# zju3dv/object_nerf

Hardware: NVIDIA H100
Metric: rays/s (higher is better)
Workload: dtype bf16

## Files before the change

object_nerf_b200/csrc/field_pe.cuh:

```cuda
#pragma once
#include "tc_common.cuh"

namespace tc {

__device__ __forceinline__ uint32_t a_chunk_addr(uint32_t base, int row, int chunk) {
  return base + (uint32_t)(chunk >> 3) * ATOM_BYTES + (uint32_t)row * 128u + (uint32_t)(((chunk & 7) ^ (row & 7)) << 4);
}
__device__ __forceinline__ void st_chunk(uint32_t addr, uint32_t a, uint32_t b, uint32_t c, uint32_t d) {
  asm volatile("st.shared.v4.b32 [%0], {%1, %2, %3, %4};" ::"r"(addr), "r"(a), "r"(b), "r"(c), "r"(d) : "memory");
}

__device__ __forceinline__ void pe8_to_chunks(uint32_t xbase, int row, int chunk0, int stride, const float* f) {
  float s[8], c[8];
  st_chunk(a_chunk_addr(xbase, row, chunk0), pack_bf16(f[0], f[1]), pack_bf16(f[2], f[3]), pack_bf16(f[4], f[5]),
           pack_bf16(f[6], f[7]));
#pragma unroll
  for (int j = 0; j < 8; ++j) __sincosf(f[j], &s[j], &c[j]);
#pragma unroll
  for (int k = 0; k < 6; ++k) {
    st_chunk(a_chunk_addr(xbase, row, chunk0 + stride * (1 + 2 * k)), pack_bf16(s[0], s[1]), pack_bf16(s[2], s[3]),
             pack_bf16(s[4], s[5]), pack_bf16(s[6], s[7]));
    st_chunk(a_chunk_addr(xbase, row, chunk0 + stride * (2 + 2 * k)), pack_bf16(c[0], c[1]), pack_bf16(c[2], c[3]),
             pack_bf16(c[4], c[5]), pack_bf16(c[6], c[7]));
    if (k < 5) {
#pragma unroll
      for (int j = 0; j < 8; ++j) {
        const float s2 = 2.0f * s[j] * c[j];
        c[j] = fmaf(-2.0f * s[j], s[j], 1.0f);
        s[j] = s2;
      }
    }
  }
}

__device__ __forceinline__ void pe_xyz_to_chunks(uint32_t xbase, int row, int chunk0, float x, float y, float z) {
  uint32_t pk[32];
  float pend = 0.0f;
  int pos = 0;
  auto emit = [&](float val) {
    if ((pos & 1) == 0) pend = val;
    else pk[pos >> 1] = pack_bf16(pend, val);
    ++pos;
  };
  emit(x); emit(y); emit(z);
  float s[3], c[3];
  sincosf(x, &s[0], &c[0]);
  sincosf(y, &s[1], &c[1]);
  sincosf(z, &s[2], &c[2]);
#pragma unroll
  for (int k = 0; k < 10; ++k) {
    emit(s[0]); emit(s[1]); emit(s[2]);
    emit(c[0]); emit(c[1]); emit(c[2]);
    if (k < 9) {
#pragma unroll
      for (int j = 0; j < 3; ++j) {
        const float s2 = 2.0f * s[j] * c[j];
        c[j] = fmaf(-2.0f * s[j], s[j], 1.0f);
        s[j] = s2;
      }
    }
  }
  emit(0.0f);
#pragma unroll
  for (int q = 0; q < 8; ++q)
    st_chunk(a_chunk_addr(xbase, row, chunk0 + q), pk[4 * q], pk[4 * q + 1], pk[4 * q + 2], pk[4 * q + 3]);
}


}
```

object_nerf_b200/csrc/field_tc.cu:

```cuda
#include <cuda_bf16.h>

#include "encode.cuh"
#include "field_common.cuh"
#include "tc_chain.cuh"
#include "field_pe.cuh"

namespace {

using namespace tc;

constexpr float kLeaky = 0.01f;

enum Epi { EPI_HIDDEN = 0, EPI_HIDDEN_RC = 1, EPI_HIDDEN_SIGMA = 2, EPI_FINAL = 3, EPI_DIR = 4 };

struct TcParams {
  FieldParams f;
  WLayer layers[MAX_LAYERS];
  int n_layers;
  uint8_t* dump;
  TrainLayout TL;
  uint32_t* diag;
};

struct RowMeta {
  int ray, si, mute, live;
};

struct Rows {
  int row[2];
  int live[2];
  int ray[2], si[2], mute[2];
  const float* rc[2];
  int64_t tile;
};

__device__ __forceinline__ uint32_t leaky_bf16x2(uint32_t x) {
  __nv_bfloat162 v = *reinterpret_cast<__nv_bfloat162*>(&x);
  const __nv_bfloat162 slope = __floats2bfloat162_rn(kLeaky, kLeaky);
  v = __hmax2(v, __hmul2(v, slope));
  return *reinterpret_cast<uint32_t*>(&v);
}

template <int N>
__device__ __forceinline__ void dump_layer(const TcParams& P, const Rows& R, int slot, int mask_word0, const uint32_t* pk) {
  const int q = threadIdx.x & 3;
#pragma unroll
  for (int r = 0; r < 2; ++r) {
    const int row = R.row[r];
    uint8_t* base = P.dump + P.TL.act_off[slot] + ((size_t)R.tile * P.TL.act_atoms[slot]) * ATOM_BYTES + (size_t)row * 128 + q * 4;
#pragma unroll
    for (int j = 0; j < N / 8; ++j)
      *reinterpret_cast<uint32_t*>(base + (size_t)(j >> 3) * ATOM_BYTES + (((j & 7) ^ (row & 7)) << 4)) = pk[2 * j + r];
  }
  if (mask_word0 < 0) return;
  constexpr int CPW = N >= 128 ? 32 : 16, NW = N / CPW, BPW = CPW / 8;
  uint32_t* mrow = reinterpret_cast<uint32_t*>(P.dump + P.TL.mask_off) + ((size_t)R.tile * ONERF_MASK_WORDS + mask_word0) * 128;
#pragma unroll
  for (int w = 0; w < NW; ++w) {
#pragma unroll
    for (int r = 0; r < 2; ++r) {
      uint32_t m = 0;
#pragma unroll
      for (int jj = 0; jj < BPW; ++jj) {
        const uint32_t v = pk[2 * (w * BPW + jj) + r];
        const uint32_t bits = (((v >> 15) & 1u) ^ 1u) | ((((v >> 31) & 1u) ^ 1u) << 1);
        m |= bits << (8 * jj + 2 * q);
      }
      m |= __shfl_xor_sync(0xffffffffu, m, 1);
      m |= __shfl_xor_sync(0xffffffffu, m, 2);
      if (q == 0) mrow[w * 128 + R.row[r]] = m;
    }
  }
}

template <int N, int EPI>
__device__ __forceinline__ void epilogue(const float (&acc)[N / 2], uint32_t* pk, const float* bias, const Rows& R,
                                         int rc_base, const float* headw, float (&part)[2][4]) {
  const int q = threadIdx.x & 3;
#pragma unroll
  for (int j = 0; j < N / 8; ++j) {
    const int c = 8 * j + 2 * q;
    float2 b[2];
    if (EPI == EPI_HIDDEN_RC || EPI == EPI_DIR) {
      b[0] = __ldg(reinterpret_cast<const float2*>(R.rc[0] + rc_base + c));
      b[1] = __ldg(reinterpret_cast<const float2*>(R.rc[1] + rc_base + c));
    } else {
      b[0] = b[1] = *reinterpret_cast<const float2*>(bias + c);
    }
#pragma unroll
    for (int r = 0; r < 2; ++r) {
      float t0 = acc[4 * j + 2 * r] + b[r].x, t1 = acc[4 * j + 2 * r + 1] + b[r].y;
      uint32_t p;
      if (EPI == EPI_HIDDEN || EPI == EPI_HIDDEN_RC) {
        p = leaky_bf16x2(pack_bf16(t0, t1));
      } else if (EPI == EPI_FINAL) {
        p = pack_bf16(t0, t1);
      } else {
        t0 = fmaxf(t0, t0 * kLeaky);
        t1 = fmaxf(t1, t1 * kLeaky);
        if (EPI == EPI_HIDDEN_SIGMA) {
          const float2 w = __ldg(reinterpret_cast<const float2*>(headw + c));
          part[r][0] = fmaf(t1, w.y, fmaf(t0, w.x, part[r][0]));
        } else {
#pragma unroll
          for (int k = 0; k < 3; ++k) {
            const float2 w = __ldg(reinterpret_cast<const float2*>(headw + k * N + c));
            part[r][1 + k] = fmaf(t1, w.y, fmaf(t0, w.x, part[r][1 + k]));
          }
        }
        p = pack_bf16(t0, t1);
      }
      pk[2 * j + r] = p;
    }
  }
}

__device__ __forceinline__ void write_heads(const FieldParams& p, const Rows& R, int branch, float (&part)[2][4]) {
  const float* Pf = reinterpret_cast<const float*>(p.packed);
  const float* hb = Pf + (branch ? p.L.orgb_b : p.L.rgb_b);
  const float sb = __ldg(Pf + (branch ? p.L.osigma_b : p.L.sigma_b));
#pragma unroll
  for (int r = 0; r < 2; ++r) {
#pragma unroll
    for (int k = 0; k < 4; ++k) {
      part[r][k] += __shfl_xor_sync(0xffffffffu, part[r][k], 1);
      part[r][k] += __shfl_xor_sync(0xffffffffu, part[r][k], 2);
    }
    if ((threadIdx.x & 3) == 0 && R.live[r]) {
      float sg = part[r][0] + sb;
      const float cr = 1.0f / (1.0f + __expf(-(part[r][1] + __ldg(hb + 0))));
      const float cg = 1.0f / (1.0f + __expf(-(part[r][2] + __ldg(hb + 1))));
      const float cb = 1.0f / (1.0f + __expf(-(part[r][3] + __ldg(hb + 2))));
      if (R.mute[r] & (branch ? 2 : 1)) sg = -1e5f;
      float* outp = branch ? p.obj_out : p.scene_out;
      reinterpret_cast<float4*>(outp)[(int64_t)R.ray[r] * p.out_stride + R.si[r]] = make_float4(cr, cg, cb, sg);
    }
  }
}

template <bool VOXEL, bool DUMP>
__global__ void __launch_bounds__(NUM_THREADS, 1) field_tc_kernel(const __grid_constant__ TcParams P) {
  extern __shared__ __align__(1024) uint8_t smem_raw[];
  const FieldParams& p = P.f;
  const int warp = threadIdx.x >> 5, lane = threadIdx.x & 31;
  constexpr int X_ATOMS = VOXEL ? 6 : 1;
  constexpr int XS = VOXEL ? 9 : 2, XO = VOXEL ? 12 : 2;

  const uint32_t sbase = (smem_u32(smem_raw) + 1023u) & ~1023u;
  const uint32_t sX = sbase;
  const uint32_t sB = sX + X_ATOMS * ATOM_BYTES;
  const uint32_t sBias = sB + NSTAGE * STAGE_BYTES;
  const uint32_t sMeta = sBias + G_COUNT * 256 * 4;
  const uint32_t sBar = sMeta + TM * sizeof(RowMeta);
  uint8_t* gen_base = smem_raw + (sbase - smem_u32(smem_raw));
  float* bias_tab = reinterpret_cast<float*>(gen_base + (sBias - sbase));
  RowMeta* meta = reinterpret_cast<RowMeta*>(gen_base + (sMeta - sbase));
  const float* Pf = reinterpret_cast<const float*>(p.packed);
  Ring ring{sB, sBar, sBar + 8 * NSTAGE, 0u, 0u, P.diag};

  if (threadIdx.x == 0) ring_init_bars(ring.full, ring.empty);
  for (int i = threadIdx.x; i < G_COUNT * 256; i += NUM_THREADS) {
    const int g = i >> 8, c = i & 255;
    bias_tab[i] = (c < p.L.g[g].N) ? __ldg(Pf + p.L.g[g].bias_off + c) : 0.0f;
  }
  __syncthreads();

  const int64_t total = (int64_t)p.n_rays * p.S;
  const int64_t n_tiles = (total + TM - 1) / TM;

  if (warp >= PRODUCER_WARP) {
    setmaxnreg_dec<PRODUCER_REGS>();
    if (warp == PRODUCER_WARP)
      tc_producer_loop(P.layers, P.n_layers, reinterpret_cast<const uint8_t*>(p.packed), ring, n_tiles);
    return;
  }
  setmaxnreg_inc<CONSUMER_REGS>();

  const int wg = warp >> 2, tid = threadIdx.x & 127;
  const uint32_t sXw = sX + (uint32_t)wg * 64u * 128u;
  Rows R;
  R.row[0] = wg * 64 + (warp & 3) * 16 + (lane >> 2);
  R.row[1] = R.row[0] + 8;
  for (int64_t tile = blockIdx.x; tile < n_tiles; tile += gridDim.x) {
    R.tile = tile;
#pragma unroll 1
    for (int job = tid; job < 256; job += 128) {
      const int row = wg * 64 + (job & 63), cq = job >> 6;
      const int64_t e = tile * TM + row;
      const bool live = e < total;
      const int ray = live ? (int)(e / p.S) : 0;
      const int si = live ? (int)(e - (int64_t)ray * p.S) : 0;
      const float* rr = p.rays + (int64_t)ray * 8;
      const float zz = live ? __ldg(p.z + (int64_t)ray * p.z_stride + si) : 0.0f;
      float x = fmaf(__ldg(rr + 3), zz, __ldg(rr + 0));
      float y = fmaf(__ldg(rr + 4), zz, __ldg(rr + 1));
      float z = fmaf(__ldg(rr + 5), zz, __ldg(rr + 2));
      if (p.xyz && live) {
        const float* qq = p.xyz + ((int64_t)ray * p.S + si) * 3;
        x = __ldg(qq); y = __ldg(qq + 1); z = __ldg(qq + 2);
      }
      if (!live) { x = 0.f; y = 0.f; z = 0.f; }
      if (cq == 0) {
        int mute = 0;
        if (live && p.mute_zero_rays && __ldg(p.z + (int64_t)ray * p.z_stride + (p.S - 1)) == 0.0f) mute = 3;
        if (live && mute == 0 && p.n_boxes > 0 && point_in_boxes(p.boxes, p.n_boxes, x, y, z)) mute = 1;
        meta[row] = RowMeta{ray, si, mute, live ? 1 : 0};
      }
      if (VOXEL) {
        const GridView g = load_grid_view(p.grid);
        float f[8];
        if (cq == 0) {
          voxel_trilinear<0, 8, false>(g, x, y, z, f);
          pe8_to_chunks(sX, row, 0, 2, f);
        } else if (cq == 1) {
          voxel_trilinear<8, 8, false>(g, x, y, z, f);
          pe8_to_chunks(sX, row, 1, 2, f);
        } else if (cq == 2) {
          voxel_trilinear<16, 8, false>(g, x, y, z, f);
          pe8_to_chunks(sX, row, 34, 1, f);
        } else {
          pe_xyz_to_chunks(sX, row, 26, x, y, z);
          st_chunk(a_chunk_addr(sX, row, 47), 0u, 0u, 0u, 0u);
        }
      } else {
        if (cq == 0) pe_xyz_to_chunks(sX, row, 0, x, y, z);
      }
    }
    fence_async_smem();
    wg_sync(wg);
    if (DUMP) {
#pragma unroll 1
      for (int a = 0; a < X_ATOMS; ++a) {
        const uint4* src = reinterpret_cast<const uint4*>(gen_base + (size_t)a * ATOM_BYTES + (size_t)wg * 8192);
        uint4* dst = reinterpret_cast<uint4*>(P.dump + P.TL.act_off[0] + ((size_t)tile * X_ATOMS + a) * ATOM_BYTES + (size_t)wg * 8192);
        for (int i = tid; i < 512; i += 128) dst[i] = src[i];
      }
    }
#pragma unroll
    for (int r = 0; r < 2; ++r) {
      const RowMeta m = meta[R.row[r]];
      R.live[r] = m.live; R.ray[r] = m.ray; R.si[r] = m.si; R.mute[r] = m.mute;
      R.rc[r] = p.ray_const + (int64_t)m.ray * ONERF_RAY_CONST_FLOATS;
    }

    if (p.want_scene) {
      float acc[128];
      uint32_t h[64];
      float part[2][4] = {};
      const float* sw = Pf + p.L.sigma_w;
      mma_layer<256, XS, 0>(acc, h, sXw, ring);
      epilogue<256, EPI_HIDDEN>(acc, h, bias_tab + G_S0 * 256, R, 0, nullptr, part);
      if (DUMP) dump_layer<256>(P, R, 1, onerf_mask_word0(1), h);
#pragma unroll 1
      for (int l = 1; l < 4; ++l) {
        mma_layer<256, 0, 8>(acc, h, sXw, ring);
        epilogue<256, EPI_HIDDEN>(acc, h, bias_tab + (G_S0 + l) * 256, R, 0, nullptr, part);
        if (DUMP) dump_layer<256>(P, R, 1 + l, onerf_mask_word0(1 + l), h);
      }
      mma_layer<256, XS, 8>(acc, h, sXw, ring);
      epilogue<256, EPI_HIDDEN>(acc, h, bias_tab + G_S4 * 256, R, 0, nullptr, part);
      if (DUMP) dump_layer<256>(P, R, 5, onerf_mask_word0(5), h);
#pragma unroll 1
      for (int l = 5; l < 7; ++l) {
        mma_layer<256, 0, 8>(acc, h, sXw, ring);
        epilogue<256, EPI_HIDDEN>(acc, h, bias_tab + (G_S0 + l) * 256, R, 0, nullptr, part);
        if (DUMP) dump_layer<256>(P, R, 1 + l, onerf_mask_word0(1 + l), h);
      }
      mma_layer<256, 0, 8>(acc, h, sXw, ring);
      epilogue<256, EPI_HIDDEN_SIGMA>(acc, h, bias_tab + G_S7 * 256, R, 0, sw, part);
      if (DUMP) dump_layer<256>(P, R, 8, onerf_mask_word0(8), h);
      mma_layer<256, 0, 8>(acc, h, sXw, ring);
      epilogue<256, EPI_FINAL>(acc, h, bias_tab + G_SFIN * 256, R, 0, nullptr, part);
      if (DUMP) dump_layer<256>(P, R, 9, -1, h);
      float accd[64];
      uint32_t hd[32];
      mma_layer<128, 0, 8>(accd, h, sXw, ring);
      epilogue<128, EPI_DIR>(accd, hd, nullptr, R, RC_SDIR, Pf + p.L.rgb_w, part);
      if (DUMP) dump_layer<128>(P, R, 10, onerf_mask_word0(10), hd);
      write_heads(p, R, 0, part);
    }
    if (p.want_object) {
      float acc[64];
      uint32_t h[32];
      float part[2][4] = {};
      mma_layer<128, XO, 0>(acc, h, sXw, ring);
      epilogue<128, EPI_HIDDEN_RC>(acc, h, nullptr, R, RC_OL0, nullptr, part);
      if (DUMP) dump_layer<128>(P, R, 11, onerf_mask_word0(11), h);
      mma_layer<128, 0, 4>(acc, h, sXw, ring);
      epilogue<128, EPI_HIDDEN>(acc, h, bias_tab + G_O1 * 256, R, 0, nullptr, part);
      if (DUMP) dump_layer<128>(P, R, 12, onerf_mask_word0(12), h);
      mma_layer<128, XO, 4>(acc, h, sXw, ring);
      epilogue<128, EPI_HIDDEN_RC>(acc, h, nullptr, R, RC_OL2, nullptr, part);
      if (DUMP) dump_layer<128>(P, R, 13, onerf_mask_word0(13), h);
      mma_layer<128, 0, 4>(acc, h, sXw, ring);
      epilogue<128, EPI_HIDDEN_SIGMA>(acc, h, bias_tab + G_O3 * 256, R, 0, Pf + p.L.osigma_w, part);
      if (DUMP) dump_layer<128>(P, R, 14, onerf_mask_word0(14), h);
      mma_layer<128, 0, 4>(acc, h, sXw, ring);
      epilogue<128, EPI_FINAL>(acc, h, bias_tab + G_OFIN * 256, R, 0, nullptr, part);
      if (DUMP) dump_layer<128>(P, R, 15, -1, h);
      float accd[32];
      uint32_t hd[16];
      mma_layer<64, 0, 4>(accd, h, sXw, ring);
      epilogue<64, EPI_DIR>(accd, hd, nullptr, R, RC_ODIR, Pf + p.L.orgb_w, part);
      if (DUMP) dump_layer<64>(P, R, 16, onerf_mask_word0(16), hd);
      write_heads(p, R, 1, part);
    }
    wg_sync(wg);
  }
}

}

int onerf_launch_field_bf16(onerf_ctx* ctx, const FieldParams& fp, cudaStream_t stream) {
  const PackLayout& L = fp.L;
  TcParams P;
  memset(&P, 0, sizeof(P));
  P.f = fp;
  int n = 0;
  auto add = [&](int g) { P.layers[n++] = WLayer{L.g[g].img_off, L.g[g].N, L.g[g].K / 32}; };
  if (fp.want_scene)
    for (int g = G_S0; g <= G_SDIR; ++g) add(g);
  if (fp.want_object)
    for (int g = G_O0; g <= G_ODIR; ++g) add(g);
  P.n_layers = n;
  P.diag = ctx->tc_diag;
  const int64_t total = (int64_t)fp.n_rays * fp.S;
  const int64_t tiles = (total + TM - 1) / TM;
  if (fp.train_ws) {
    P.dump = reinterpret_cast<uint8_t*>(fp.train_ws);
    P.TL = onerf_make_train_layout(L.use_voxel, total);
  }
  const int blocks = (int)(tiles < ctx->num_sms ? tiles : ctx->num_sms);
  const int x_atoms = L.use_voxel ? 6 : 1;
  const size_t smem = 1024 + (size_t)x_atoms * ATOM_BYTES + NSTAGE * STAGE_BYTES + G_COUNT * 256 * 4 + TM * sizeof(RowMeta) +
                      16 * NSTAGE;
  auto launch = [&](auto kernel) -> int {
    ONERF_CUDA(cudaFuncSetAttribute(kernel, cudaFuncAttributeMaxDynamicSharedMemorySize, (int)smem));
    kernel<<<blocks, NUM_THREADS, smem, stream>>>(P);
    ONERF_LAUNCH_CHECK(ctx);
    return ONERF_OK;
  };
  if (L.use_voxel) return fp.train_ws ? launch(field_tc_kernel<true, true>) : launch(field_tc_kernel<true, false>);
  return fp.train_ws ? launch(field_tc_kernel<false, true>) : launch(field_tc_kernel<false, false>);
}
```

object_nerf_b200/csrc/tc_chain.cuh:

```cuda
#pragma once
#include "tc_common.cuh"

namespace tc {

constexpr int NSTAGE = 6;
constexpr int STAGE_BYTES = 16384;
constexpr int NUM_WG = 2;
constexpr int NUM_CONSUMER = NUM_WG * 128;
constexpr int PRODUCER_WARP = NUM_CONSUMER / 32;
constexpr int NUM_THREADS = NUM_CONSUMER + 128;
constexpr int PRODUCER_REGS = 40, CONSUMER_REGS = 232;
constexpr int MAX_LAYERS = 16;

struct WLayer {
  int64_t img_off;
  int N;
  int nslab;
};

struct Ring {
  uint32_t sB, full, empty;
  uint32_t stage, phase;
  uint32_t* diag;
};

__device__ __forceinline__ void ring_init_bars(uint32_t full, uint32_t empty) {
  for (int s = 0; s < NSTAGE; ++s) {
    mbar_init(full + 8 * s, 1);
    mbar_init(empty + 8 * s, NUM_CONSUMER / 32);
  }
  fence_barrier_init();
}

__device__ __forceinline__ void tc_producer_loop(const WLayer* layers, int n_layers, const uint8_t* blob, Ring r,
                                                 int64_t n_tiles) {
  for (int64_t tile = blockIdx.x; tile < n_tiles; tile += gridDim.x) {
    for (int l = 0; l < n_layers; ++l) {
      const WLayer& Ly = layers[l];
      const int spp = 256 / Ly.N;
      const uint32_t slab_bytes = (uint32_t)Ly.N * 64u;
      for (int s0 = 0; s0 < Ly.nslab; s0 += spp) {
        const int cnt = (Ly.nslab - s0 < spp) ? Ly.nslab - s0 : spp;
        mbar_wait(r.empty + 8 * r.stage, r.phase ^ 1, r.diag);
        if (elect_one()) {
          mbar_expect_tx(r.full + 8 * r.stage, (uint32_t)cnt * slab_bytes);
          tma_bulk_g2s(r.sB + r.stage * STAGE_BYTES, blob + Ly.img_off + (size_t)s0 * slab_bytes, (uint32_t)cnt * slab_bytes,
                       r.full + 8 * r.stage);
        }
        __syncwarp();
        if (++r.stage == NSTAGE) { r.stage = 0; r.phase ^= 1; }
      }
    }
  }
}

__device__ __forceinline__ void ring_release(const Ring& r, uint32_t stage) {
  asm volatile(
      "{\n\t.reg .pred p;\n\tsetp.eq.u32 p, %1, 0;\n\t@p mbarrier.arrive.shared::cta.b64 _, [%0];\n\t}" ::"r"(
          r.empty + 8 * stage),
      "r"(threadIdx.x & 31)
      : "memory");
}

template <int N, int NX, int NH, int W = N>
__device__ __forceinline__ void mma_layer(float (&acc)[N / 2], const uint32_t* hin, uint32_t sXw, Ring& r) {
  constexpr int SPP = 256 / N, NS = NX + NH;
#pragma unroll
  for (int i = 0; i < N / 2; ++i) acc[i] = 0.0f;
  uint32_t prev = 0;
#pragma unroll
  for (int s = 0; s < NS; ++s) {
    if (s % SPP == 0) mbar_wait(r.full + 8 * r.stage, r.phase, r.diag);
    const uint32_t b0 = r.sB + r.stage * STAGE_BYTES + (uint32_t)(s % SPP) * (uint32_t)N * 64u;
    wgmma_fence();
#pragma unroll
    for (int k16 = 0; k16 < 2; ++k16) {
#pragma unroll
      for (int nb = 0; nb < N / W; ++nb) {
        const uint64_t bd = desc_k_sw64(b0 + (uint32_t)nb * (uint32_t)W * 64u + (uint32_t)k16 * 32u);
        if (s < NX)
          wgmma_ss<W>(acc + nb * (W / 2),
                      desc_k_sw128(sXw + (uint32_t)(s >> 1) * ATOM_BYTES + (uint32_t)(s & 1) * 64u + (uint32_t)k16 * 32u), bd);
        else
          wgmma_rs<W>(acc + nb * (W / 2), hin + ((s - NX) * 2 + k16) * 4, bd);
      }
    }
    if (s % SPP == SPP - 1 || s == NS - 1) {
      wgmma_commit();
      if (s >= SPP) {
        wgmma_wait<1>();
        ring_release(r, prev);
      }
      prev = r.stage;
      if (++r.stage == NSTAGE) { r.stage = 0; r.phase ^= 1; }
    }
  }
  wgmma_wait<0>();
  ring_release(r, prev);
  fence_regs<N / 2>(acc);
}

}
```

object_nerf_b200/csrc/tc_common.cuh:

```cuda
#pragma once
#include <cuda_bf16.h>
#include <stdint.h>

namespace tc {

constexpr int TM = 128;
constexpr int ATOM_BYTES = 16384;

__device__ __forceinline__ uint32_t smem_u32(const void* p) { return (uint32_t)__cvta_generic_to_shared(p); }

__device__ __forceinline__ void mbar_init(uint32_t bar, uint32_t count) {
  asm volatile("mbarrier.init.shared::cta.b64 [%0], %1;" ::"r"(bar), "r"(count));
}
__device__ __forceinline__ void mbar_arrive(uint32_t bar) {
  asm volatile("mbarrier.arrive.shared::cta.b64 _, [%0];" ::"r"(bar) : "memory");
}
__device__ __forceinline__ void mbar_expect_tx(uint32_t bar, uint32_t bytes) {
  asm volatile("mbarrier.arrive.expect_tx.shared::cta.b64 _, [%0], %1;" ::"r"(bar), "r"(bytes) : "memory");
}
__device__ __forceinline__ void mbar_wait(uint32_t bar, uint32_t parity, uint32_t* diag) {
  asm volatile(
      "{\n\t.reg .pred p;\n\t.reg .u64 t0, t1;\n\t.reg .u32 b;\n\t"
      "mbarrier.try_wait.parity.shared::cta.b64 p, [%0], %1, %2;\n\t"
      "@p bra DONE;\n\t"
      "mov.u64 t0, %%clock64;\n"
      "WAIT:\n\t"
      "mbarrier.try_wait.parity.shared::cta.b64 p, [%0], %1, %2;\n\t"
      "@p bra DONE;\n\t"
      "mov.u64 t1, %%clock64;\n\t"
      "sub.u64 t1, t1, t0;\n\t"
      "setp.lt.u64 p, t1, %4;\n\t"
      "@p bra WAIT;\n\t"
      "mov.u32 b, %%ctaid.x;\n\t"
      "st.volatile.u32 [%3 + 4], b;\n\t"
      "st.volatile.u32 [%3 + 8], %0;\n\t"
      "st.volatile.u32 [%3 + 12], %1;\n\t"
      "membar.sys;\n\t"
      "st.volatile.u32 [%3], 1;\n\t"
      "membar.sys;\n\t"
      "trap;\n"
      "DONE:\n\t}"
      :
      : "r"(bar), "r"(parity), "r"(20000u), "l"(diag), "n"(4000000000ll)
      : "memory");
}
__device__ __forceinline__ void fence_barrier_init() { asm volatile("fence.mbarrier_init.release.cluster;" ::: "memory"); }
__device__ __forceinline__ void fence_async_smem() { asm volatile("fence.proxy.async.shared::cta;" ::: "memory"); }

__device__ __forceinline__ void tma_bulk_g2s(uint32_t dst, const void* src, uint32_t bytes, uint32_t bar) {
  asm volatile("cp.async.bulk.shared::cluster.global.mbarrier::complete_tx::bytes [%0], [%1], %2, [%3];" ::"r"(dst),
               "l"(src), "r"(bytes), "r"(bar)
               : "memory");
}

__device__ __forceinline__ bool elect_one() {
  uint32_t pred;
  asm volatile(
      "{\n\t.reg .pred p;\n\t"
      "elect.sync _|p, 0xffffffff;\n\t"
      "selp.u32 %0, 1, 0, p;\n\t}"
      : "=r"(pred));
  return pred != 0;
}

template <int N>
__device__ __forceinline__ void setmaxnreg_dec() { asm volatile("setmaxnreg.dec.sync.aligned.u32 %0;" ::"n"(N)); }
template <int N>
__device__ __forceinline__ void setmaxnreg_inc() { asm volatile("setmaxnreg.inc.sync.aligned.u32 %0;" ::"n"(N)); }

__device__ __forceinline__ void wg_sync(int wg) { asm volatile("bar.sync %0, 128;" ::"r"(1 + wg) : "memory"); }

__device__ __forceinline__ void wgmma_fence() { asm volatile("wgmma.fence.sync.aligned;" ::: "memory"); }
__device__ __forceinline__ void wgmma_commit() { asm volatile("wgmma.commit_group.sync.aligned;" ::: "memory"); }
template <int N>
__device__ __forceinline__ void wgmma_wait() { asm volatile("wgmma.wait_group.sync.aligned %0;" ::"n"(N) : "memory"); }

template <int NR>
__device__ __forceinline__ void fence_regs(float* d) {
#pragma unroll
  for (int i = 0; i < NR; ++i) asm volatile("" : "+f"(d[i])::"memory");
}

#define ONERF_WG_D32                                                                                                   \
  "{%0, %1, %2, %3, %4, %5, %6, %7, %8, %9, %10, %11, %12, %13, %14, %15, %16, %17, %18, %19, %20, %21, %22, %23, %24, " \
  "%25, %26, %27, %28, %29, %30, %31}"
#define ONERF_WG_OUT32(d)                                                                                              \
  "+f"((d)[0]), "+f"((d)[1]), "+f"((d)[2]), "+f"((d)[3]), "+f"((d)[4]), "+f"((d)[5]), "+f"((d)[6]), "+f"((d)[7]),      \
      "+f"((d)[8]), "+f"((d)[9]), "+f"((d)[10]), "+f"((d)[11]), "+f"((d)[12]), "+f"((d)[13]), "+f"((d)[14]),           \
      "+f"((d)[15]), "+f"((d)[16]), "+f"((d)[17]), "+f"((d)[18]), "+f"((d)[19]), "+f"((d)[20]), "+f"((d)[21]),         \
      "+f"((d)[22]), "+f"((d)[23]), "+f"((d)[24]), "+f"((d)[25]), "+f"((d)[26]), "+f"((d)[27]), "+f"((d)[28]),         \
      "+f"((d)[29]), "+f"((d)[30]), "+f"((d)[31])
#define ONERF_WG_OUT64(d) ONERF_WG_OUT32(d), ONERF_WG_OUT32((d) + 32)
#define ONERF_WG_OUT128(d) ONERF_WG_OUT64(d), ONERF_WG_OUT64((d) + 64)
#define ONERF_WG_D64 "{" \
  "%0, %1, %2, %3, %4, %5, %6, %7, %8, %9, %10, %11, %12, %13, %14, %15, " \
  "%16, %17, %18, %19, %20, %21, %22, %23, %24, %25, %26, %27, %28, %29, %30, %31, " \
  "%32, %33, %34, %35, %36, %37, %38, %39, %40, %41, %42, %43, %44, %45, %46, %47, " \
  "%48, %49, %50, %51, %52, %53, %54, %55, %56, %57, %58, %59, %60, %61, %62, %63" "}"
#define ONERF_WG_D128 "{" \
  "%0, %1, %2, %3, %4, %5, %6, %7, %8, %9, %10, %11, %12, %13, %14, %15, " \
  "%16, %17, %18, %19, %20, %21, %22, %23, %24, %25, %26, %27, %28, %29, %30, %31, " \
  "%32, %33, %34, %35, %36, %37, %38, %39, %40, %41, %42, %43, %44, %45, %46, %47, " \
  "%48, %49, %50, %51, %52, %53, %54, %55, %56, %57, %58, %59, %60, %61, %62, %63, " \
  "%64, %65, %66, %67, %68, %69, %70, %71, %72, %73, %74, %75, %76, %77, %78, %79, " \
  "%80, %81, %82, %83, %84, %85, %86, %87, %88, %89, %90, %91, %92, %93, %94, %95, " \
  "%96, %97, %98, %99, %100, %101, %102, %103, %104, %105, %106, %107, %108, %109, %110, %111, " \
  "%112, %113, %114, %115, %116, %117, %118, %119, %120, %121, %122, %123, %124, %125, %126, %127" "}"

__device__ __forceinline__ void wgmma_rs_n64(float* d, const uint32_t* a, uint64_t desc_b) {
  asm volatile(
      "{\n\t.reg .pred p;\n\tsetp.ne.b32 p, %37, 0;\n\t"
      "wgmma.mma_async.sync.aligned.m64n64k16.f32.bf16.bf16 " ONERF_WG_D32 ", {%32, %33, %34, %35}, %36, p, 1, 1, 0;\n\t}"
      : ONERF_WG_OUT32(d)
      : "r"(a[0]), "r"(a[1]), "r"(a[2]), "r"(a[3]), "l"(desc_b), "r"(1));
}
template <int TA, int TB>
__device__ __forceinline__ void wgmma_ss_n64(float* d, uint64_t desc_a, uint64_t desc_b) {
  asm volatile(
      "{\n\t.reg .pred p;\n\tsetp.ne.b32 p, %34, 0;\n\t"
      "wgmma.mma_async.sync.aligned.m64n64k16.f32.bf16.bf16 " ONERF_WG_D32 ", %32, %33, p, 1, 1, %35, %36;\n\t}"
      : ONERF_WG_OUT32(d)
      : "l"(desc_a), "l"(desc_b), "r"(1), "n"(TA), "n"(TB));
}

template <int N>
__device__ __forceinline__ void wgmma_rs(float* d, const uint32_t* a, uint64_t desc_b) {
  if constexpr (N == 64) {
    wgmma_rs_n64(d, a, desc_b);
  } else if constexpr (N == 128) {
    asm volatile(
        "{\n\t.reg .pred p;\n\tsetp.ne.b32 p, %69, 0;\n\t"
        "wgmma.mma_async.sync.aligned.m64n128k16.f32.bf16.bf16 " ONERF_WG_D64 ", {%64, %65, %66, %67}, %68, p, 1, 1, 0;\n\t}"
        : ONERF_WG_OUT64(d)
        : "r"(a[0]), "r"(a[1]), "r"(a[2]), "r"(a[3]), "l"(desc_b), "r"(1));
  } else {
    static_assert(N == 256, "wgmma_rs: N is 64, 128 or 256");
    asm volatile(
        "{\n\t.reg .pred p;\n\tsetp.ne.b32 p, %133, 0;\n\t"
        "wgmma.mma_async.sync.aligned.m64n256k16.f32.bf16.bf16 " ONERF_WG_D128 ", {%128, %129, %130, %131}, %132, p, 1, 1, 0;\n\t}"
        : ONERF_WG_OUT128(d)
        : "r"(a[0]), "r"(a[1]), "r"(a[2]), "r"(a[3]), "l"(desc_b), "r"(1));
  }
}
template <int N>
__device__ __forceinline__ void wgmma_ss(float* d, uint64_t desc_a, uint64_t desc_b) {
  if constexpr (N == 64) {
    wgmma_ss_n64<0, 0>(d, desc_a, desc_b);
  } else if constexpr (N == 128) {
    asm volatile(
        "{\n\t.reg .pred p;\n\tsetp.ne.b32 p, %66, 0;\n\t"
        "wgmma.mma_async.sync.aligned.m64n128k16.f32.bf16.bf16 " ONERF_WG_D64 ", %64, %65, p, 1, 1, 0, 0;\n\t}"
        : ONERF_WG_OUT64(d)
        : "l"(desc_a), "l"(desc_b), "r"(1));
  } else {
    static_assert(N == 256, "wgmma_ss: N is 64, 128 or 256");
    asm volatile(
        "{\n\t.reg .pred p;\n\tsetp.ne.b32 p, %130, 0;\n\t"
        "wgmma.mma_async.sync.aligned.m64n256k16.f32.bf16.bf16 " ONERF_WG_D128 ", %128, %129, p, 1, 1, 0, 0;\n\t}"
        : ONERF_WG_OUT128(d)
        : "l"(desc_a), "l"(desc_b), "r"(1));
  }
}

__device__ __forceinline__ uint64_t make_desc(uint32_t saddr, uint32_t lbo_bytes, uint32_t sbo_bytes, uint32_t layout) {
  return (uint64_t)((saddr >> 4) & 0x3FFFu) | ((uint64_t)((lbo_bytes >> 4) & 0x3FFFu) << 16) |
         ((uint64_t)((sbo_bytes >> 4) & 0x3FFFu) << 32) | ((uint64_t)layout << 62);
}
__device__ __forceinline__ uint64_t desc_k_sw128(uint32_t saddr) { return make_desc(saddr, 16, 1024, 1); }
__device__ __forceinline__ uint64_t desc_k_sw64(uint32_t saddr) { return make_desc(saddr, 16, 512, 2); }
__device__ __forceinline__ uint64_t desc_mn_sw128(uint32_t saddr, uint32_t lbo_bytes) { return make_desc(saddr, lbo_bytes, 1024, 1); }

__device__ __forceinline__ uint32_t pack_bf16(float lo, float hi) {
  __nv_bfloat162 t = __floats2bfloat162_rn(lo, hi);
  return *reinterpret_cast<uint32_t*>(&t);
}
__device__ __forceinline__ float bf16_lo(uint32_t w) { return __uint_as_float(w << 16); }
__device__ __forceinline__ float bf16_hi(uint32_t w) { return __uint_as_float(w & 0xffff0000u); }

__device__ __forceinline__ uint32_t atom_chunk_off(int row, int chunk) {
  return (uint32_t)(chunk >> 3) * ATOM_BYTES + (uint32_t)row * 128u + (uint32_t)(((chunk & 7) ^ (row & 7)) << 4);
}


}
```

Before: 1.463 million.

## Move input encoding to dedicated encoder warps with mbarrier handoff and prefetch

```diff
diff --git a/object_nerf_b200/csrc/field_pe.cuh b/object_nerf_b200/csrc/field_pe.cuh
--- a/object_nerf_b200/csrc/field_pe.cuh
+++ b/object_nerf_b200/csrc/field_pe.cuh
@@ -34,12 +34,13 @@
 }
 
 __device__ __forceinline__ void pe_xyz_to_chunks(uint32_t xbase, int row, int chunk0, float x, float y, float z) {
-  uint32_t pk[32];
+  uint32_t pk[4];
   float pend = 0.0f;
   int pos = 0;
   auto emit = [&](float val) {
     if ((pos & 1) == 0) pend = val;
-    else pk[pos >> 1] = pack_bf16(pend, val);
+    else pk[(pos >> 1) & 3] = pack_bf16(pend, val);
+    if ((pos & 7) == 7) st_chunk(a_chunk_addr(xbase, row, chunk0 + (pos >> 3)), pk[0], pk[1], pk[2], pk[3]);
     ++pos;
   };
   emit(x); emit(y); emit(z);
@@ -61,9 +62,6 @@
     }
   }
   emit(0.0f);
-#pragma unroll
-  for (int q = 0; q < 8; ++q)
-    st_chunk(a_chunk_addr(xbase, row, chunk0 + q), pk[4 * q], pk[4 * q + 1], pk[4 * q + 2], pk[4 * q + 3]);
 }
 
 
diff --git a/object_nerf_b200/csrc/field_tc.cu b/object_nerf_b200/csrc/field_tc.cu
--- a/object_nerf_b200/csrc/field_tc.cu
+++ b/object_nerf_b200/csrc/field_tc.cu
@@ -20,6 +20,9 @@
   uint8_t* dump;
   TrainLayout TL;
   uint32_t* diag;
+#ifdef ONERF_FIELD_TIMELINE
+  uint64_t* tl;
+#endif
 };
 
 struct RowMeta {
@@ -32,7 +35,30 @@
   int ray[2], si[2], mute[2];
   const float* rc[2];
   int64_t tile;
+#ifdef ONERF_FIELD_TIMELINE
+  uint64_t* tl;
+#endif
 };
+
+#ifdef ONERF_FIELD_TIMELINE
+constexpr int TL_CTAS = 8, TL_TILES = 16, TL_SLOTS = 80;
+uint64_t* g_timeline = nullptr;
+__device__ __forceinline__ void tl_put(uint64_t* tl, int slot, uint64_t v) {
+  asm volatile("{\n\t.reg .pred p;\n\tsetp.ne.u64 p, %0, 0;\n\t@p st.global.u64 [%1], %2;\n\t}" ::"l"(tl), "l"(tl + slot),
+               "l"(v)
+               : "memory");
+}
+__device__ __forceinline__ uint64_t* tl_record(const TcParams& P, int64_t tile, int wg, bool lead) {
+  const int64_t k = (tile - blockIdx.x) / gridDim.x;
+  if (!P.tl || !lead || blockIdx.x >= TL_CTAS || k >= TL_TILES) return nullptr;
+  return P.tl + (((int64_t)blockIdx.x * 3 + wg) * TL_TILES + k) * TL_SLOTS;
+}
+#define TL_AT(tl, slot) tl_put((tl), (slot), clock64())
+#define TL_PUT(tl, slot, v) tl_put((tl), (slot), (v))
+#else
+#define TL_AT(tl, slot)
+#define TL_PUT(tl, slot, v)
+#endif
 
 __device__ __forceinline__ uint32_t leaky_bf16x2(uint32_t x) {
   __nv_bfloat162 v = *reinterpret_cast<__nv_bfloat162*>(&x);
@@ -138,54 +164,69 @@
   }
 }
 
-template <bool VOXEL, bool DUMP>
-__global__ void __launch_bounds__(NUM_THREADS, 1) field_tc_kernel(const __grid_constant__ TcParams P) {
-  extern __shared__ __align__(1024) uint8_t smem_raw[];
+__device__ __forceinline__ void x_release(uint32_t x_free, bool on) {
+  asm volatile(
+      "{\n\t.reg .pred p;\n\tsetp.eq.u32 p, %1, 1;\n\t@p mbarrier.arrive.shared::cta.b64 _, [%0];\n\t}" ::"r"(x_free),
+      "r"((uint32_t)on & (uint32_t)((threadIdx.x & 31) == 0))
+      : "memory");
+}
+
+template <int N, int NX, int NH, int EPI, bool DUMP>
+__device__ __forceinline__ void run_layer(const TcParams& P, const Rows& R, Ring& ring, uint32_t sXw, float (&acc)[N / 2],
+                                          const uint32_t* hin, uint32_t* hout, const float* bias, int rc_base,
+                                          const float* headw, float (&part)[2][4], int slot, int mask_word0,
+                                          uint32_t x_free = 0, bool free_x = false) {
+  TL_AT(R.tl, 3 * slot);
+  mma_layer<N, NX, NH>(acc, hin, sXw, ring);
+  if constexpr (NX > 0) x_release(x_free, free_x);
+  TL_AT(R.tl, 3 * slot + 1);
+#ifdef ONERF_FIELD_TIMELINE
+  TL_PUT(R.tl, 55 + slot, ring.full_wait);
+  ring.full_wait = 0;
+#endif
+  epilogue<N, EPI>(acc, hout, bias, R, rc_base, headw, part);
+  if (DUMP) dump_layer<N>(P, R, slot, mask_word0, hout);
+  TL_AT(R.tl, 3 * slot + 2);
+}
+
+constexpr int NUM_ENCODER = 3 * 32;
+
+__device__ __forceinline__ void prefetch_l2(const void* ptr) {
+  asm volatile("prefetch.global.L2 [%0];" ::"l"(ptr));
+}
+
+__device__ __forceinline__ void prefetch_rows(const void* base, int64_t pitch, int64_t bytes0, int nbytes, int r0,
+                                              int r1, int et) {
+  const int lines = (nbytes + 127) >> 7;
+  for (int i = et; i < (r1 - r0 + 1) * lines; i += NUM_ENCODER)
+    prefetch_l2(reinterpret_cast<const char*>(base) + (r0 + i / lines) * pitch + bytes0 + (int64_t)(i % lines) * 128);
+}
+
+template <bool VOXEL>
+__device__ __forceinline__ void encoder_loop(const TcParams& P, uint32_t sX, RowMeta* meta, uint32_t x_full,
+                                             uint32_t x_free, int64_t n_tiles, int64_t total) {
   const FieldParams& p = P.f;
-  const int warp = threadIdx.x >> 5, lane = threadIdx.x & 31;
-  constexpr int X_ATOMS = VOXEL ? 6 : 1;
-  constexpr int XS = VOXEL ? 9 : 2, XO = VOXEL ? 12 : 2;
-
-  const uint32_t sbase = (smem_u32(smem_raw) + 1023u) & ~1023u;
-  const uint32_t sX = sbase;
-  const uint32_t sB = sX + X_ATOMS * ATOM_BYTES;
-  const uint32_t sBias = sB + NSTAGE * STAGE_BYTES;
-  const uint32_t sMeta = sBias + G_COUNT * 256 * 4;
-  const uint32_t sBar = sMeta + TM * sizeof(RowMeta);
-  uint8_t* gen_base = smem_raw + (sbase - smem_u32(smem_raw));
-  float* bias_tab = reinterpret_cast<float*>(gen_base + (sBias - sbase));
-  RowMeta* meta = reinterpret_cast<RowMeta*>(gen_base + (sMeta - sbase));
-  const float* Pf = reinterpret_cast<const float*>(p.packed);
-  Ring ring{sB, sBar, sBar + 8 * NSTAGE, 0u, 0u, P.diag};
-
-  if (threadIdx.x == 0) ring_init_bars(ring.full, ring.empty);
-  for (int i = threadIdx.x; i < G_COUNT * 256; i += NUM_THREADS) {
-    const int g = i >> 8, c = i & 255;
-    bias_tab[i] = (c < p.L.g[g].N) ? __ldg(Pf + p.L.g[g].bias_off + c) : 0.0f;
-  }
-  __syncthreads();
-
-  const int64_t total = (int64_t)p.n_rays * p.S;
-  const int64_t n_tiles = (total + TM - 1) / TM;
-
-  if (warp >= PRODUCER_WARP) {
-    setmaxnreg_dec<PRODUCER_REGS>();
-    if (warp == PRODUCER_WARP)
-      tc_producer_loop(P.layers, P.n_layers, reinterpret_cast<const uint8_t*>(p.packed), ring, n_tiles);
-    return;
-  }
-  setmaxnreg_inc<CONSUMER_REGS>();
-
-  const int wg = warp >> 2, tid = threadIdx.x & 127;
-  const uint32_t sXw = sX + (uint32_t)wg * 64u * 128u;
-  Rows R;
-  R.row[0] = wg * 64 + (warp & 3) * 16 + (lane >> 2);
-  R.row[1] = R.row[0] + 8;
-  for (int64_t tile = blockIdx.x; tile < n_tiles; tile += gridDim.x) {
-    R.tile = tile;
+  const int et = threadIdx.x - NUM_CONSUMER - 32;
+  constexpr int JOBS = VOXEL ? 4 * TM : TM;
+  uint32_t it = 0;
+  for (int64_t tile = blockIdx.x; tile < n_tiles; tile += gridDim.x, ++it) {
+#ifdef ONERF_FIELD_TIMELINE
+    uint64_t* tl = tl_record(P, tile, 2, et == 0);
+#endif
+    TL_AT(tl, 0);
+    {
+      const int64_t e0 = tile * TM, e1 = min(e0 + TM, total) - 1;
+      prefetch_rows(p.ray_const, ONERF_RAY_CONST_FLOATS * 4, 0, ONERF_RAY_CONST_FLOATS * 4, (int)(e0 / p.S),
+                    (int)(e1 / p.S), et);
+      const int64_t n0 = e0 + (int64_t)gridDim.x * TM, n1 = min(n0 + TM, total) - 1;
+      if (n0 < total) {
+        prefetch_rows(p.rays, 32, 0, 32, (int)(n0 / p.S), (int)(n1 / p.S), et);
+        prefetch_rows(p.z, p.z_stride * 4, 0, p.S * 4, (int)(n0 / p.S), (int)(n1 / p.S), et);
+      }
+    }
 #pragma unroll 1
-    for (int job = tid; job < 256; job += 128) {
-      const int row = wg * 64 + (job & 63), cq = job >> 6;
+    for (int job = et; job < JOBS; job += NUM_ENCODER) {
+      const int row = job & (TM - 1), cq = job / TM;
       const int64_t e = tile * TM + row;
       const bool live = e < total;
       const int ray = live ? (int)(e / p.S) : 0;
@@ -204,30 +245,91 @@
         int mute = 0;
         if (live && p.mute_zero_rays && __ldg(p.z + (int64_t)ray * p.z_stride + (p.S - 1)) == 0.0f) mute = 3;
         if (live && mute == 0 && p.n_boxes > 0 && point_in_boxes(p.boxes, p.n_boxes, x, y, z)) mute = 1;
+        mbar_wait(x_free, (it & 1) ^ 1, P.diag);
         meta[row] = RowMeta{ray, si, mute, live ? 1 : 0};
       }
-      if (VOXEL) {
+      if (VOXEL && cq < 3) {
         const GridView g = load_grid_view(p.grid);
         float f[8];
-        if (cq == 0) {
-          voxel_trilinear<0, 8, false>(g, x, y, z, f);
-          pe8_to_chunks(sX, row, 0, 2, f);
-        } else if (cq == 1) {
-          voxel_trilinear<8, 8, false>(g, x, y, z, f);
-          pe8_to_chunks(sX, row, 1, 2, f);
-        } else if (cq == 2) {
-          voxel_trilinear<16, 8, false>(g, x, y, z, f);
-          pe8_to_chunks(sX, row, 34, 1, f);
-        } else {
-          pe_xyz_to_chunks(sX, row, 26, x, y, z);
-          st_chunk(a_chunk_addr(sX, row, 47), 0u, 0u, 0u, 0u);
-        }
-      } else {
-        if (cq == 0) pe_xyz_to_chunks(sX, row, 0, x, y, z);
-      }
-    }
+        if (cq == 0) voxel_trilinear<0, 8, false>(g, x, y, z, f);
+        else if (cq == 1) voxel_trilinear<8, 8, false>(g, x, y, z, f);
+        else voxel_trilinear<16, 8, false>(g, x, y, z, f);
+        mbar_wait(x_free, (it & 1) ^ 1, P.diag);
+        pe8_to_chunks(sX, row, cq < 2 ? cq : 34, cq < 2 ? 2 : 1, f);
+      } else if (cq == (VOXEL ? 3 : 0)) {
+        mbar_wait(x_free, (it & 1) ^ 1, P.diag);
+        pe_xyz_to_chunks(sX, row, VOXEL ? 26 : 0, x, y, z);
+        if (VOXEL) st_chunk(a_chunk_addr(sX, row, 47), 0u, 0u, 0u, 0u);
+      }
+    }
+    mbar_wait(x_free, (it & 1) ^ 1, P.diag);
+    TL_AT(tl, 1);
     fence_async_smem();
-    wg_sync(wg);
+    mbar_arrive(x_full);
+    TL_AT(tl, 2);
+  }
+}
+
+template <bool VOXEL, bool DUMP>
+__global__ void __launch_bounds__(NUM_THREADS, 1) field_tc_kernel(const __grid_constant__ TcParams P) {
+  extern __shared__ __align__(1024) uint8_t smem_raw[];
+  const FieldParams& p = P.f;
+  const int warp = threadIdx.x >> 5, lane = threadIdx.x & 31;
+  constexpr int X_ATOMS = VOXEL ? 6 : 1;
+  constexpr int XS = VOXEL ? 9 : 2, XO = VOXEL ? 12 : 2;
+
+  const uint32_t sbase = (smem_u32(smem_raw) + 1023u) & ~1023u;
+  const uint32_t sX = sbase;
+  const uint32_t sB = sX + X_ATOMS * ATOM_BYTES;
+  const uint32_t sBias = sB + NSTAGE * STAGE_BYTES;
+  const uint32_t sMeta = sBias + G_COUNT * 256 * 4;
+  const uint32_t sBar = sMeta + TM * sizeof(RowMeta);
+  const uint32_t x_full = sBar + 16 * NSTAGE, x_free = x_full + 8;
+  uint8_t* gen_base = smem_raw + (sbase - smem_u32(smem_raw));
+  float* bias_tab = reinterpret_cast<float*>(gen_base + (sBias - sbase));
+  RowMeta* meta = reinterpret_cast<RowMeta*>(gen_base + (sMeta - sbase));
+  const float* Pf = reinterpret_cast<const float*>(p.packed);
+  Ring ring{sB, sBar, sBar + 8 * NSTAGE, 0u, 0u, P.diag};
+
+  if (threadIdx.x == 0) {
+    mbar_init(x_full, NUM_ENCODER);
+    mbar_init(x_free, NUM_CONSUMER / 32);
+    ring_init_bars(ring.full, ring.empty);
+  }
+  for (int i = threadIdx.x; i < G_COUNT * 256; i += NUM_THREADS) {
+    const int g = i >> 8, c = i & 255;
+    bias_tab[i] = (c < p.L.g[g].N) ? __ldg(Pf + p.L.g[g].bias_off + c) : 0.0f;
+  }
+  __syncthreads();
+
+  const int64_t total = (int64_t)p.n_rays * p.S;
+  const int64_t n_tiles = (total + TM - 1) / TM;
+
+  if (warp >= PRODUCER_WARP) {
+    setmaxnreg_dec<PRODUCER_REGS>();
+    if (warp == PRODUCER_WARP)
+      tc_producer_loop(P.layers, P.n_layers, reinterpret_cast<const uint8_t*>(p.packed), ring, n_tiles);
+    else
+      encoder_loop<VOXEL>(P, sX, meta, x_full, x_free, n_tiles, total);
+    return;
+  }
+  setmaxnreg_inc<CONSUMER_REGS>();
+
+  const int wg = warp >> 2, tid = threadIdx.x & 127;
+  const uint32_t sXw = sX + (uint32_t)wg * 64u * 128u;
+  const bool free_after_o2 = !p.want_scene;
+  Rows R;
+  R.row[0] = wg * 64 + (warp & 3) * 16 + (lane >> 2);
+  R.row[1] = R.row[0] + 8;
+  uint32_t it = 0;
+  for (int64_t tile = blockIdx.x; tile < n_tiles; tile += gridDim.x, ++it) {
+    R.tile = tile;
+#ifdef ONERF_FIELD_TIMELINE
+    R.tl = tl_record(P, tile, wg, tid == 0);
+#endif
+    TL_AT(R.tl, 0);
+    mbar_wait(x_full, it & 1, P.diag);
+    TL_AT(R.tl, 1);
     if (DUMP) {
 #pragma unroll 1
       for (int a = 0; a < X_ATOMS; ++a) {
@@ -242,70 +344,55 @@
       R.live[r] = m.live; R.ray[r] = m.ray; R.si[r] = m.si; R.mute[r] = m.mute;
       R.rc[r] = p.ray_const + (int64_t)m.ray * ONERF_RAY_CONST_FLOATS;
     }
-
+    TL_AT(R.tl, 2);
+
+    if (p.want_object) {
+      float acc[64];
+      uint32_t h[32];
+      float part[2][4] = {};
+      run_layer<128, XO, 0, EPI_HIDDEN_RC, DUMP>(P, R, ring, sXw, acc, h, h, nullptr, RC_OL0, nullptr, part, 11,
+                                                 onerf_mask_word0(11), x_free, false);
+      run_layer<128, 0, 4, EPI_HIDDEN, DUMP>(P, R, ring, sXw, acc, h, h, bias_tab + G_O1 * 256, 0, nullptr, part, 12,
+                                             onerf_mask_word0(12));
+      run_layer<128, XO, 4, EPI_HIDDEN_RC, DUMP>(P, R, ring, sXw, acc, h, h, nullptr, RC_OL2, nullptr, part, 13,
+                                                 onerf_mask_word0(13), x_free, free_after_o2);
+      run_layer<128, 0, 4, EPI_HIDDEN_SIGMA, DUMP>(P, R, ring, sXw, acc, h, h, bias_tab + G_O3 * 256, 0,
+                                                   Pf + p.L.osigma_w, part, 14, onerf_mask_word0(14));
+      run_layer<128, 0, 4, EPI_FINAL, DUMP>(P, R, ring, sXw, acc, h, h, bias_tab + G_OFIN * 256, 0, nullptr, part, 15, -1);
+      float accd[32];
+      uint32_t hd[16];
+      run_layer<64, 0, 4, EPI_DIR, DUMP>(P, R, ring, sXw, accd, h, hd, nullptr, RC_ODIR, Pf + p.L.orgb_w, part, 16,
+                                         onerf_mask_word0(16));
+      write_heads(p, R, 1, part);
+    }
     if (p.want_scene) {
       float acc[128];
       uint32_t h[64];
       float part[2][4] = {};
       const float* sw = Pf + p.L.sigma_w;
-      mma_layer<256, XS, 0>(acc, h, sXw, ring);
-      epilogue<256, EPI_HIDDEN>(acc, h, bias_tab + G_S0 * 256, R, 0, nullptr, part);
-      if (DUMP) dump_layer<256>(P, R, 1, onerf_mask_word0(1), h);
+      run_layer<256, XS, 0, EPI_HIDDEN, DUMP>(P, R, ring, sXw, acc, h, h, bias_tab + G_S0 * 256, 0, nullptr, part, 1,
+                                              onerf_mask_word0(1), x_free, false);
 #pragma unroll 1
-      for (int l = 1; l < 4; ++l) {
-        mma_layer<256, 0, 8>(acc, h, sXw, ring);
-        epilogue<256, EPI_HIDDEN>(acc, h, bias_tab + (G_S0 + l) * 256, R, 0, nullptr, part);
-        if (DUMP) dump_layer<256>(P, R, 1 + l, onerf_mask_word0(1 + l), h);
-      }
-      mma_layer<256, XS, 8>(acc, h, sXw, ring);
-      epilogue<256, EPI_HIDDEN>(acc, h, bias_tab + G_S4 * 256, R, 0, nullptr, part);
-      if (DUMP) dump_layer<256>(P, R, 5, onerf_mask_word0(5), h);
+      for (int l = 1; l < 4; ++l)
+        run_layer<256, 0, 8, EPI_HIDDEN, DUMP>(P, R, ring, sXw, acc, h, h, bias_tab + (G_S0 + l) * 256, 0, nullptr, part,
+                                               1 + l, onerf_mask_word0(1 + l));
+      run_layer<256, XS, 8, EPI_HIDDEN, DUMP>(P, R, ring, sXw, acc, h, h, bias_tab + G_S4 * 256, 0, nullptr, part, 5,
+                                              onerf_mask_word0(5), x_free, true);
 #pragma unroll 1
-      for (int l = 5; l < 7; ++l) {
-        mma_layer<256, 0, 8>(acc, h, sXw, ring);
-        epilogue<256, EPI_HIDDEN>(acc, h, bias_tab + (G_S0 + l) * 256, R, 0, nullptr, part);
-        if (DUMP) dump_layer<256>(P, R, 1 + l, onerf_mask_word0(1 + l), h);
-      }
-      mma_layer<256, 0, 8>(acc, h, sXw, ring);
-      epilogue<256, EPI_HIDDEN_SIGMA>(acc, h, bias_tab + G_S7 * 256, R, 0, sw, part);
-      if (DUMP) dump_layer<256>(P, R, 8, onerf_mask_word0(8), h);
-      mma_layer<256, 0, 8>(acc, h, sXw, ring);
-      epilogue<256, EPI_FINAL>(acc, h, bias_tab + G_SFIN * 256, R, 0, nullptr, part);
-      if (DUMP) dump_layer<256>(P, R, 9, -1, h);
+      for (int l = 5; l < 7; ++l)
+        run_layer<256, 0, 8, EPI_HIDDEN, DUMP>(P, R, ring, sXw, acc, h, h, bias_tab + (G_S0 + l) * 256, 0, nullptr, part,
+                                               1 + l, onerf_mask_word0(1 + l));
+      run_layer<256, 0, 8, EPI_HIDDEN_SIGMA, DUMP>(P, R, ring, sXw, acc, h, h, bias_tab + G_S7 * 256, 0, sw, part, 8,
+                                                   onerf_mask_word0(8));
+      run_layer<256, 0, 8, EPI_FINAL, DUMP>(P, R, ring, sXw, acc, h, h, bias_tab + G_SFIN * 256, 0, nullptr, part, 9, -1);
       float accd[64];
       uint32_t hd[32];
-      mma_layer<128, 0, 8>(accd, h, sXw, ring);
-      epilogue<128, EPI_DIR>(accd, hd, nullptr, R, RC_SDIR, Pf + p.L.rgb_w, part);
-      if (DUMP) dump_layer<128>(P, R, 10, onerf_mask_word0(10), hd);
+      run_layer<128, 0, 8, EPI_DIR, DUMP>(P, R, ring, sXw, accd, h, hd, nullptr, RC_SDIR, Pf + p.L.rgb_w, part, 10,
+                                          onerf_mask_word0(10));
       write_heads(p, R, 0, part);
     }
-    if (p.want_object) {
-      float acc[64];
-      uint32_t h[32];
-      float part[2][4] = {};
-      mma_layer<128, XO, 0>(acc, h, sXw, ring);
-      epilogue<128, EPI_HIDDEN_RC>(acc, h, nullptr, R, RC_OL0, nullptr, part);
-      if (DUMP) dump_layer<128>(P, R, 11, onerf_mask_word0(11), h);
-      mma_layer<128, 0, 4>(acc, h, sXw, ring);
-      epilogue<128, EPI_HIDDEN>(acc, h, bias_tab + G_O1 * 256, R, 0, nullptr, part);
-      if (DUMP) dump_layer<128>(P, R, 12, onerf_mask_word0(12), h);
-      mma_layer<128, XO, 4>(acc, h, sXw, ring);
-      epilogue<128, EPI_HIDDEN_RC>(acc, h, nullptr, R, RC_OL2, nullptr, part);
-      if (DUMP) dump_layer<128>(P, R, 13, onerf_mask_word0(13), h);
-      mma_layer<128, 0, 4>(acc, h, sXw, ring);
-      epilogue<128, EPI_HIDDEN_SIGMA>(acc, h, bias_tab + G_O3 * 256, R, 0, Pf + p.L.osigma_w, part);
-      if (DUMP) dump_layer<128>(P, R, 14, onerf_mask_word0(14), h);
-      mma_layer<128, 0, 4>(acc, h, sXw, ring);
-      epilogue<128, EPI_FINAL>(acc, h, bias_tab + G_OFIN * 256, R, 0, nullptr, part);
-      if (DUMP) dump_layer<128>(P, R, 15, -1, h);
-      float accd[32];
-      uint32_t hd[16];
-      mma_layer<64, 0, 4>(accd, h, sXw, ring);
-      epilogue<64, EPI_DIR>(accd, hd, nullptr, R, RC_ODIR, Pf + p.L.orgb_w, part);
-      if (DUMP) dump_layer<64>(P, R, 16, onerf_mask_word0(16), hd);
-      write_heads(p, R, 1, part);
-    }
-    wg_sync(wg);
+    TL_AT(R.tl, 51);
+    TL_AT(R.tl, 52);
   }
 }
 
@@ -318,12 +405,15 @@
   P.f = fp;
   int n = 0;
   auto add = [&](int g) { P.layers[n++] = WLayer{L.g[g].img_off, L.g[g].N, L.g[g].K / 32}; };
+  if (fp.want_object)
+    for (int g = G_O0; g <= G_ODIR; ++g) add(g);
   if (fp.want_scene)
     for (int g = G_S0; g <= G_SDIR; ++g) add(g);
-  if (fp.want_object)
-    for (int g = G_O0; g <= G_ODIR; ++g) add(g);
   P.n_layers = n;
   P.diag = ctx->tc_diag;
+#ifdef ONERF_FIELD_TIMELINE
+  P.tl = g_timeline;
+#endif
   const int64_t total = (int64_t)fp.n_rays * fp.S;
   const int64_t tiles = (total + TM - 1) / TM;
   if (fp.train_ws) {
@@ -333,7 +423,7 @@
   const int blocks = (int)(tiles < ctx->num_sms ? tiles : ctx->num_sms);
   const int x_atoms = L.use_voxel ? 6 : 1;
   const size_t smem = 1024 + (size_t)x_atoms * ATOM_BYTES + NSTAGE * STAGE_BYTES + G_COUNT * 256 * 4 + TM * sizeof(RowMeta) +
-                      16 * NSTAGE;
+                      16 * NSTAGE + 16;
   auto launch = [&](auto kernel) -> int {
     ONERF_CUDA(cudaFuncSetAttribute(kernel, cudaFuncAttributeMaxDynamicSharedMemorySize, (int)smem));
     kernel<<<blocks, NUM_THREADS, smem, stream>>>(P);
@@ -343,3 +433,7 @@
   if (L.use_voxel) return fp.train_ws ? launch(field_tc_kernel<true, true>) : launch(field_tc_kernel<true, false>);
   return fp.train_ws ? launch(field_tc_kernel<false, true>) : launch(field_tc_kernel<false, false>);
 }
+
+#ifdef ONERF_FIELD_TIMELINE
+extern "C" void onerf_field_timeline(void* buf) { g_timeline = static_cast<uint64_t*>(buf); }
+#endif
diff --git a/object_nerf_b200/csrc/tc_chain.cuh b/object_nerf_b200/csrc/tc_chain.cuh
--- a/object_nerf_b200/csrc/tc_chain.cuh
+++ b/object_nerf_b200/csrc/tc_chain.cuh
@@ -22,6 +22,9 @@
   uint32_t sB, full, empty;
   uint32_t stage, phase;
   uint32_t* diag;
+#ifdef ONERF_FIELD_TIMELINE
+  uint64_t full_wait = 0;
+#endif
 };
 
 __device__ __forceinline__ void ring_init_bars(uint32_t full, uint32_t empty) {
@@ -65,12 +68,18 @@
 template <int N, int NX, int NH, int W = N>
 __device__ __forceinline__ void mma_layer(float (&acc)[N / 2], const uint32_t* hin, uint32_t sXw, Ring& r) {
   constexpr int SPP = 256 / N, NS = NX + NH;
-#pragma unroll
-  for (int i = 0; i < N / 2; ++i) acc[i] = 0.0f;
   uint32_t prev = 0;
 #pragma unroll
   for (int s = 0; s < NS; ++s) {
-    if (s % SPP == 0) mbar_wait(r.full + 8 * r.stage, r.phase, r.diag);
+    if (s % SPP == 0) {
+#ifdef ONERF_FIELD_TIMELINE
+      const uint64_t t0 = clock64();
+#endif
+      mbar_wait(r.full + 8 * r.stage, r.phase, r.diag);
+#ifdef ONERF_FIELD_TIMELINE
+      r.full_wait += clock64() - t0;
+#endif
+    }
     const uint32_t b0 = r.sB + r.stage * STAGE_BYTES + (uint32_t)(s % SPP) * (uint32_t)N * 64u;
     wgmma_fence();
 #pragma unroll
@@ -78,11 +87,13 @@
 #pragma unroll
       for (int nb = 0; nb < N / W; ++nb) {
         const uint64_t bd = desc_k_sw64(b0 + (uint32_t)nb * (uint32_t)W * 64u + (uint32_t)k16 * 32u);
+        const int scale_d = (s == 0 && k16 == 0) ? 0 : 1;
         if (s < NX)
           wgmma_ss<W>(acc + nb * (W / 2),
-                      desc_k_sw128(sXw + (uint32_t)(s >> 1) * ATOM_BYTES + (uint32_t)(s & 1) * 64u + (uint32_t)k16 * 32u), bd);
+                      desc_k_sw128(sXw + (uint32_t)(s >> 1) * ATOM_BYTES + (uint32_t)(s & 1) * 64u + (uint32_t)k16 * 32u), bd,
+                      scale_d);
         else
-          wgmma_rs<W>(acc + nb * (W / 2), hin + ((s - NX) * 2 + k16) * 4, bd);
+          wgmma_rs<W>(acc + nb * (W / 2), hin + ((s - NX) * 2 + k16) * 4, bd, scale_d);
       }
     }
     if (s % SPP == SPP - 1 || s == NS - 1) {
diff --git a/object_nerf_b200/csrc/tc_common.cuh b/object_nerf_b200/csrc/tc_common.cuh
--- a/object_nerf_b200/csrc/tc_common.cuh
+++ b/object_nerf_b200/csrc/tc_common.cuh
@@ -68,8 +68,6 @@
 template <int N>
 __device__ __forceinline__ void setmaxnreg_inc() { asm volatile("setmaxnreg.inc.sync.aligned.u32 %0;" ::"n"(N)); }
 
-__device__ __forceinline__ void wg_sync(int wg) { asm volatile("bar.sync %0, 128;" ::"r"(1 + wg) : "memory"); }
-
 __device__ __forceinline__ void wgmma_fence() { asm volatile("wgmma.fence.sync.aligned;" ::: "memory"); }
 __device__ __forceinline__ void wgmma_commit() { asm volatile("wgmma.commit_group.sync.aligned;" ::: "memory"); }
 template <int N>
@@ -107,58 +105,58 @@
   "%96, %97, %98, %99, %100, %101, %102, %103, %104, %105, %106, %107, %108, %109, %110, %111, " \
   "%112, %113, %114, %115, %116, %117, %118, %119, %120, %121, %122, %123, %124, %125, %126, %127" "}"
 
-__device__ __forceinline__ void wgmma_rs_n64(float* d, const uint32_t* a, uint64_t desc_b) {
+__device__ __forceinline__ void wgmma_rs_n64(float* d, const uint32_t* a, uint64_t desc_b, int scale_d = 1) {
   asm volatile(
       "{\n\t.reg .pred p;\n\tsetp.ne.b32 p, %37, 0;\n\t"
       "wgmma.mma_async.sync.aligned.m64n64k16.f32.bf16.bf16 " ONERF_WG_D32 ", {%32, %33, %34, %35}, %36, p, 1, 1, 0;\n\t}"
       : ONERF_WG_OUT32(d)
-      : "r"(a[0]), "r"(a[1]), "r"(a[2]), "r"(a[3]), "l"(desc_b), "r"(1));
+      : "r"(a[0]), "r"(a[1]), "r"(a[2]), "r"(a[3]), "l"(desc_b), "r"(scale_d));
 }
 template <int TA, int TB>
-__device__ __forceinline__ void wgmma_ss_n64(float* d, uint64_t desc_a, uint64_t desc_b) {
+__device__ __forceinline__ void wgmma_ss_n64(float* d, uint64_t desc_a, uint64_t desc_b, int scale_d = 1) {
   asm volatile(
       "{\n\t.reg .pred p;\n\tsetp.ne.b32 p, %34, 0;\n\t"
       "wgmma.mma_async.sync.aligned.m64n64k16.f32.bf16.bf16 " ONERF_WG_D32 ", %32, %33, p, 1, 1, %35, %36;\n\t}"
       : ONERF_WG_OUT32(d)
-      : "l"(desc_a), "l"(desc_b), "r"(1), "n"(TA), "n"(TB));
+      : "l"(desc_a), "l"(desc_b), "r"(scale_d), "n"(TA), "n"(TB));
 }
 
 template <int N>
-__device__ __forceinline__ void wgmma_rs(float* d, const uint32_t* a, uint64_t desc_b) {
+__device__ __forceinline__ void wgmma_rs(float* d, const uint32_t* a, uint64_t desc_b, int scale_d = 1) {
   if constexpr (N == 64) {
-    wgmma_rs_n64(d, a, desc_b);
+    wgmma_rs_n64(d, a, desc_b, scale_d);
   } else if constexpr (N == 128) {
     asm volatile(
         "{\n\t.reg .pred p;\n\tsetp.ne.b32 p, %69, 0;\n\t"
         "wgmma.mma_async.sync.aligned.m64n128k16.f32.bf16.bf16 " ONERF_WG_D64 ", {%64, %65, %66, %67}, %68, p, 1, 1, 0;\n\t}"
         : ONERF_WG_OUT64(d)
-        : "r"(a[0]), "r"(a[1]), "r"(a[2]), "r"(a[3]), "l"(desc_b), "r"(1));
+        : "r"(a[0]), "r"(a[1]), "r"(a[2]), "r"(a[3]), "l"(desc_b), "r"(scale_d));
   } else {
     static_assert(N == 256, "wgmma_rs: N is 64, 128 or 256");
     asm volatile(
         "{\n\t.reg .pred p;\n\tsetp.ne.b32 p, %133, 0;\n\t"
         "wgmma.mma_async.sync.aligned.m64n256k16.f32.bf16.bf16 " ONERF_WG_D128 ", {%128, %129, %130, %131}, %132, p, 1, 1, 0;\n\t}"
         : ONERF_WG_OUT128(d)
-        : "r"(a[0]), "r"(a[1]), "r"(a[2]), "r"(a[3]), "l"(desc_b), "r"(1));
+        : "r"(a[0]), "r"(a[1]), "r"(a[2]), "r"(a[3]), "l"(desc_b), "r"(scale_d));
   }
 }
 template <int N>
-__device__ __forceinline__ void wgmma_ss(float* d, uint64_t desc_a, uint64_t desc_b) {
+__device__ __forceinline__ void wgmma_ss(float* d, uint64_t desc_a, uint64_t desc_b, int scale_d = 1) {
   if constexpr (N == 64) {
-    wgmma_ss_n64<0, 0>(d, desc_a, desc_b);
+    wgmma_ss_n64<0, 0>(d, desc_a, desc_b, scale_d);
   } else if constexpr (N == 128) {
     asm volatile(
         "{\n\t.reg .pred p;\n\tsetp.ne.b32 p, %66, 0;\n\t"
         "wgmma.mma_async.sync.aligned.m64n128k16.f32.bf16.bf16 " ONERF_WG_D64 ", %64, %65, p, 1, 1, 0, 0;\n\t}"
         : ONERF_WG_OUT64(d)
-        : "l"(desc_a), "l"(desc_b), "r"(1));
+        : "l"(desc_a), "l"(desc_b), "r"(scale_d));
   } else {
     static_assert(N == 256, "wgmma_ss: N is 64, 128 or 256");
     asm volatile(
         "{\n\t.reg .pred p;\n\tsetp.ne.b32 p, %130, 0;\n\t"
         "wgmma.mma_async.sync.aligned.m64n256k16.f32.bf16.bf16 " ONERF_WG_D128 ", %128, %129, p, 1, 1, 0, 0;\n\t}"
         : ONERF_WG_OUT128(d)
-        : "l"(desc_a), "l"(desc_b), "r"(1));
+        : "l"(desc_a), "l"(desc_b), "r"(scale_d));
   }
 }
 
```

Result: faster. 1.561 million, median of 6 (+6.7%).
